# KuldeepChoksi/video-anomaly-detection

Measured on AMD Instinct MI355X. Metric: frames/sec/GPU (256x256 autoencoder scoring) + AUROC parity vs reference, higher is better.
Workload: dtype f32; 1 GPU; configs[1]: image autoencoder scoring, batch 512 synthetic 256x256x3 frames per GPU; chunk=512, weights=deterministic synthetic state dict (Xavier scale, randomised BN), collective=none (1 GPU)

## Files before the change

### video-anomaly-detection_amd/csrc/conv_wino.hip

```cpp
#include <atomic>

#include "vad_common.h"

#define MFMA32W(a, b, c) __builtin_amdgcn_mfma_f32_32x32x2f32((a), (b), (c), 0, 0, 0)

struct ConvWP {
    const float* in;  long long in_fs;
    const float* in2; long long in2_fs;
    int cin_a;
    const float* w;
    const float* bias;
    float* out;       long long out_fs;
    int n, h, w_, cin, cout;
    int tiles_x, tiles_y, cblocks;
    const float* c_prev; float* c_out; int hid;
};

template <int NT, int POOL, int ACT>
__global__ __launch_bounds__(256, 2) void conv3x3_wino_pkernel(ConvWP p) {
    static_assert(POOL != 2 || NT == 2, "fused ConvLSTM cell: two N-tiles (i|f and g|o) per wave");
    constexpr int CK = 32, LW = 18, LH = 10, PS = CK + 4, NPIX = LW * LH;
    constexpr int TOT = NPIX * (CK / 4), NPF = (TOT + 255) / 256;
    constexpr int XF = 4 * 2 * NT * 64 * 16;
    constexpr int TILE_F = NPIX * PS;
    constexpr int SMEM = (2 * TILE_F > XF) ? 2 * TILE_F : XF;
    constexpr int NS = 16;
    constexpr int PB = 1, NB = 2;
    __shared__ __attribute__((aligned(16))) float smem[SMEM];

    const int tid = threadIdx.x, lane = tid & 63, wave = tid >> 6;
    const int li = lane & 31, lh = lane >> 5;

    const unsigned per_frame = (unsigned)(p.tiles_x * p.tiles_y * p.cblocks);
    unsigned L = vad_xcd_remap(blockIdx.x % per_frame, per_frame);
    const int fg = blockIdx.x / per_frame, fgroups = gridDim.x / per_frame;
    const int cb = L % p.cblocks; L /= p.cblocks;
    const int x0 = (L % p.tiles_x) * 16, y0 = (L / p.tiles_x) * 8;
    const int H = p.h, W = p.w_;
    const int nch_a = p.cin_a / CK;
    const int nch = (p.in2 ? p.cin : p.cin_a) / CK;

    unsigned svo[NPF];
    const int c4 = tid & 7, pix0 = tid >> 3;
#pragma unroll
    for (int i = 0; i < NPF; ++i) {
        const int pix = pix0 + 32 * i;
        const int ly = pix / LW, lx = pix - ly * LW;
        const int gy = y0 - 1 + ly, gx = x0 - 1 + lx;
        const bool ok = pix < NPIX && gy >= 0 && gy < H && gx >= 0 && gx < W;
        svo[i] = ok ? (unsigned)(__mul24(__mul24(gy, W) + gx, p.cin_a) + c4 * 4) * 4u : VAD_OOB;
    }
    const unsigned in_bytes = (unsigned)(H * W) * (unsigned)p.cin_a * 4u;
    f32x4 pf[NPF];
#define ISSUE(n_, ch_)                                                                                   \
    {                                                                                                    \
        const float* src_ = ((ch_) < nch_a) ? p.in + (size_t)(n_) * p.in_fs + (ch_) * CK                 \
                                            : p.in2 + (size_t)(n_) * p.in2_fs + ((ch_) - nch_a) * CK;    \
        const unsigned skip_ = (unsigned)(((ch_) < nch_a) ? (ch_) : (ch_) - nch_a) * CK * 4u;            \
        const __amdgpu_buffer_rsrc_t r_ = vad_rsrc(src_, in_bytes - skip_);                              \
        _Pragma("unroll") for (int i_ = 0; i_ < NPF; ++i_) pf[i_] = vad_bload4(r_, svo[i_], 0);          \
    }

    const int tr = li >> 3, tc = li & 7;
    const int ia = (wave == 0) ? 0 : (wave == 2) ? 2 : 1;
    const int ib = (wave == 0) ? 2 : (wave == 1) ? 2 : (wave == 2) ? 1 : 3;
    const float sgn = (wave == 1) ? 1.f : -1.f;
    const int rowa = ((2 * tr + ia) * LW + 2 * tc) * PS + 4 * lh;
    const int rowb = ((2 * tr + ib) * LW + 2 * tc) * PS + 4 * lh;

    const unsigned wf = (unsigned)p.cout * 32u;
    const unsigned ftap = (unsigned)(p.cin / 8) * wf;
    const __amdgpu_buffer_rsrc_t rw = vad_rsrc(p.w, 16u * ftap);
    unsigned wl[NT];
    float bv[NT];
#pragma unroll
    for (int nt = 0; nt < NT; ++nt) {
        const int co = (POOL == 2) ? (2 * nt + (li >> 4)) * p.hid + cb * 16 + (li & 15) : (cb * NT + nt) * 32 + li;
        wl[nt] = (unsigned)(wave * 4) * ftap + (unsigned)co * 32u + 16u * lh;
        bv[nt] = p.bias[co];
    }
    f32x4 b[NB][NT];
#define LOAD_B(buf, chunk, step)                                                 \
    {                                                                                                    \
        const unsigned soff_ = (unsigned)((step) & 3) * ftap + (unsigned)((chunk) * 4 + ((step) >> 2)) * wf; \
        _Pragma("unroll") for (int nt = 0; nt < NT; ++nt) b[buf][nt] = vad_bload4(rw, wl[nt], soff_);    \
    }

    const int ech = (POOL == 2) ? p.hid : p.cout;
    const int ow = (POOL == 1) ? (W >> 1) : W, oh = (POOL == 1) ? (H >> 1) : H;
    const int ey0 = (POOL == 1) ? (y0 >> 1) + wave : y0 + 2 * wave;
    const int ex0 = (POOL == 1) ? (x0 >> 1) + 4 * lh : x0 + 8 * lh;
    const unsigned erow = (unsigned)__mul24(ow, ech) * 4u, ecol = (unsigned)ech * 4u;
    const unsigned eoff = (POOL == 2) ? (unsigned)(__mul24(__mul24(ey0, ow) + ex0 + (li >> 4), ech) + cb * 16 + (li & 15)) * 4u
                                      : (unsigned)(__mul24(__mul24(ey0, ow) + ex0, ech) + cb * NT * 32 + li) * 4u;
    const unsigned out_bytes = (unsigned)__mul24(oh, ow) * (unsigned)ech * 4u;
    const bool full_tile = (y0 + 8 <= H) && (x0 + 16 <= W);
    const int sw = (lane >> 2) & 3;

    int n = fg;
    if (n >= p.n) return;
    ISSUE(n, 0);
#pragma unroll
    for (int s0 = 0; s0 < PB; ++s0) LOAD_B(s0, 0, s0);
#pragma unroll
    for (int nt = 0; nt < NT; ++nt) asm volatile("" ::"v"(bv[nt]));

    f32x16 acc[4][NT];
    const f32x16 zero16 = {0.f, 0.f, 0.f, 0.f, 0.f, 0.f, 0.f, 0.f, 0.f, 0.f, 0.f, 0.f, 0.f, 0.f, 0.f, 0.f};
#define LOAD_RAW(kg)                                                                                     \
    {                                                                                                    \
        _Pragma("unroll") for (int j_ = 0; j_ < 4; ++j_) {                                               \
            raw[0][j_] = *(const f32x4*)&tile_[rowa + j_ * PS + (kg) * 8];                               \
            raw[1][j_] = *(const f32x4*)&tile_[rowb + j_ * PS + (kg) * 8];                               \
        }                                                                                                \
    }
#define TRANSFORM_V()                                                                                    \
    {                                                                                                    \
        f32x4 t_[4];                                                                                     \
        _Pragma("unroll") for (int j_ = 0; j_ < 4; ++j_)                                                 \
            _Pragma("unroll") for (int e_ = 0; e_ < 4; ++e_) t_[j_][e_] = __builtin_fmaf(sgn, raw[1][j_][e_], raw[0][j_][e_]); \
        v[0] = t_[0] - t_[2];                                                                            \
        v[1] = t_[1] + t_[2];                                                                            \
        v[2] = t_[2] - t_[1];                                                                            \
        v[3] = t_[1] - t_[3];                                                                            \
    }
#define CHUNK(FIRST, ch, n_, nn_, has_next_)                                                             \
    {                                                                                                    \
                                       \
        float* tile_ = smem + (((ch) & 1) ? TILE_F : 0);                                                 \
        _Pragma("unroll") for (int i = 0; i < NPF; ++i)                                                  \
            if (pix0 + 32 * i < NPIX) *(f32x4*)&tile_[(pix0 + 32 * i) * PS + c4 * 4] = pf[i];            \
        __syncthreads();                                                                                 \
        f32x4 raw[2][4], v[4];                                 \
        LOAD_RAW(0);                                                                                     \
        if ((ch) + 1 < nch) { ISSUE(n_, (ch) + 1); }                                                     \
        else if (has_next_) { ISSUE(nn_, 0); }                                                           \
        TRANSFORM_V();                                                                                   \
        _Pragma("unroll") for (int kg = 0; kg < 4; ++kg) {                                               \
            if (kg + 1 < 4) { LOAD_RAW(kg + 1); }                                                        \
            _Pragma("unroll") for (int fc = 0; fc < 4; ++fc) {                                           \
                const int s_ = kg * 4 + fc, bcur = s_ % NB, bnxt = (s_ + PB) % NB;                       \
                if (s_ + PB < NS) { LOAD_B(bnxt, ch, s_ + PB); }                                         \
                else if ((ch) + 1 < nch) { LOAD_B(bnxt, (ch) + 1, s_ + PB - NS); }                       \
                __builtin_amdgcn_sched_barrier(0);                                                       \
                _Pragma("unroll") for (int j = 0; j < 4; ++j)                                            \
                    _Pragma("unroll") for (int nt = 0; nt < NT; ++nt)                                    \
                        acc[fc][nt] = MFMA32W(v[fc][j], b[bcur][nt][j], ((FIRST) && kg == 0 && j == 0) ? zero16 : acc[fc][nt]); \
                __builtin_amdgcn_sched_barrier(0);                                                       \
            }                                                                                            \
            if (kg + 1 < 4) { TRANSFORM_V(); }                                                           \
        }                                                                                                \
    }

    while (true) {
        const int nn = n + fgroups;
        const bool has_next = nn < p.n;
        CHUNK(1, 0, n, nn, has_next);
        for (int ch = 1; ch < nch; ++ch) CHUNK(0, ch, n, nn, has_next);

        f32x16 P[2][NT];
#pragma unroll
        for (int nt = 0; nt < NT; ++nt) {
            P[0][nt] = acc[0][nt] + acc[1][nt] + acc[2][nt];
            P[1][nt] = acc[1][nt] - acc[2][nt] - acc[3][nt];
        }
        if (has_next) {
#pragma unroll
            for (int s0 = 0; s0 < PB; ++s0) LOAD_B(s0, 0, s0);
        }
        __syncthreads();
#pragma unroll
        for (int j = 0; j < 2; ++j)
#pragma unroll
            for (int nt = 0; nt < NT; ++nt)
#pragma unroll
                for (int q = 0; q < 4; ++q)
                    *(f32x4*)&smem[((((wave * 2 + j) * NT + nt) * 64 + lane) * 4 + (q ^ sw)) * 4] =
                        f32x4{P[j][nt][4 * q], P[j][nt][4 * q + 1], P[j][nt][4 * q + 2], P[j][nt][4 * q + 3]};
        __syncthreads();
        const __amdgpu_buffer_rsrc_t ro = vad_rsrc(p.out + (size_t)n * p.out_fs, out_bytes);
        f32x4 yy[NT][2][2];
        float cpv[POOL == 2 ? 8 : 1];
        if constexpr (POOL == 2) {
            const __amdgpu_buffer_rsrc_t rc = vad_rsrc(p.c_prev ? p.c_prev + (size_t)n * (out_bytes / 4) : p.c_out, p.c_prev ? out_bytes : 0u);
#pragma unroll
            for (int dy = 0; dy < 2; ++dy)
#pragma unroll
                for (int kk = 0; kk < 4; ++kk) {
                    const bool ok = full_tile || ((ey0 + dy) < oh && (ex0 + 2 * kk + (li >> 4)) < ow);
                    cpv[dy * 4 + kk] = vad_bload1(rc, ok ? eoff : VAD_OOB, dy * erow + 2 * kk * ecol);
                }
        }
#pragma unroll
        for (int nt = 0; nt < NT; ++nt)
#pragma unroll
            for (int j = 0; j < 2; ++j) {
                f32x4 pr[4];
#pragma unroll
                for (int r = 0; r < 4; ++r) pr[r] = *(const f32x4*)&smem[((((r * 2 + j) * NT + nt) * 64 + lane) * 4 + (wave ^ sw)) * 4];
                yy[nt][0][j] = pr[0] + pr[1] + pr[2];
                yy[nt][1][j] = pr[1] - pr[2] - pr[3];
            }
        if constexpr (POOL == 2) {
            const bool hi = (li >> 4) != 0;
            const __amdgpu_buffer_rsrc_t rco = vad_rsrc(p.c_out + (size_t)n * (out_bytes / 4), out_bytes);
#pragma unroll
            for (int dy = 0; dy < 2; ++dy)
#pragma unroll
                for (int kk = 0; kk < 4; ++kk) {
                    float own[2], got[2];
#pragma unroll
                    for (int nt = 0; nt < 2; ++nt) {
                        const float keep = hi ? yy[nt][dy][1][kk] : yy[nt][dy][0][kk];
                        const float give = hi ? yy[nt][dy][0][kk] : yy[nt][dy][1][kk];
                        own[nt] = keep + bv[nt];
                        got[nt] = __builtin_bit_cast(float, __builtin_amdgcn_ds_swizzle(__builtin_bit_cast(int, give + bv[nt]), 0x401f));
                    }
                    const float zi = hi ? got[0] : own[0], zf = hi ? own[0] : got[0], zg = hi ? got[1] : own[1], zo = hi ? own[1] : got[1];
                    float cn, hn;
                    vad_lstm_cell(zi, zf, zg, zo, cpv[dy * 4 + kk], cn, hn);
                    const bool ok = full_tile || ((ey0 + dy) < oh && (ex0 + 2 * kk + (li >> 4)) < ow);
                    const unsigned so = dy * erow + 2 * kk * ecol;
                    vad_bstore1(cn, rco, ok ? eoff : VAD_OOB, so);
                    vad_bstore1(hn, ro, ok ? eoff : VAD_OOB, so);
                }
        } else {
#pragma unroll
            for (int nt = 0; nt < NT; ++nt) {
                if (POOL == 1) {
#pragma unroll
                    for (int kk = 0; kk < 4; ++kk) {
                        const bool ok = full_tile || (ey0 < oh && (ex0 + kk) < ow);
                        const float m = fmaxf(fmaxf(yy[nt][0][0][kk], yy[nt][0][1][kk]), fmaxf(yy[nt][1][0][kk], yy[nt][1][1][kk]));
                        vad_bstore1(vad_act(m + bv[nt], ACT), ro, ok ? eoff : VAD_OOB, kk * ecol + nt * 128u);
                    }
                } else {
#pragma unroll
                    for (int dy = 0; dy < 2; ++dy)
#pragma unroll
                        for (int kk = 0; kk < 4; ++kk)
#pragma unroll
                            for (int dx = 0; dx < 2; ++dx) {
                                const bool ok = full_tile || ((ey0 + dy) < oh && (ex0 + 2 * kk + dx) < ow);
                                vad_bstore1(vad_act(yy[nt][dy][dx][kk] + bv[nt], ACT), ro, ok ? eoff : VAD_OOB, dy * erow + (2 * kk + dx) * ecol + nt * 128u);
                            }
                }
            }
        }
        if (!has_next) break;
        n = nn;
        __syncthreads();
    }
#undef ISSUE
#undef LOAD_B
#undef CHUNK
#undef LOAD_RAW
#undef TRANSFORM_V
}

static int wino_num_cus() {
    static std::atomic<int> cached{0};
    int ncu = cached.load(std::memory_order_relaxed);
    if (!ncu) {
        int dev = 0;
        hipDeviceProp_t prop;
        if (hipGetDevice(&dev) == hipSuccess && hipGetDeviceProperties(&prop, dev) == hipSuccess) ncu = prop.multiProcessorCount;
        if (ncu <= 0) ncu = 256;
        cached = ncu;
    }
    return ncu;
}

template <int NT, int POOL, int ACT>
static void launch_wino(const ConvWP& p, hipStream_t s) {
    static std::atomic<unsigned> cap_{0};
    unsigned cap = cap_.load(std::memory_order_relaxed);
    if (!cap) {
        int per_cu = 0;
        if (hipOccupancyMaxActiveBlocksPerMultiprocessor(&per_cu, conv3x3_wino_pkernel<NT, POOL, ACT>, 256, 0) != hipSuccess || per_cu < 1) per_cu = 1;
        cap_ = cap = (unsigned)wino_num_cus() * (unsigned)per_cu;
    }
    const unsigned per_frame = (unsigned)(p.tiles_x * p.tiles_y * p.cblocks);
    unsigned fgroups = cap / per_frame;
    if (fgroups < 1) fgroups = 1;
    if (fgroups > (unsigned)p.n) fgroups = (unsigned)p.n;
    hipLaunchKernelGGL((conv3x3_wino_pkernel<NT, POOL, ACT>), dim3(per_frame * fgroups), dim3(256), 0, s, p);
}

template <int NT>
static int launch_wino_nt(const ConvWP& p, int act, int pool, hipStream_t s) {
#define W_(P_, A_) launch_wino<NT, P_, A_>(p, s)
    if (pool) { if (act == VAD_ACT_LEAKY) W_(1, VAD_ACT_LEAKY); else if (act == VAD_ACT_RELU) W_(1, VAD_ACT_RELU); else W_(1, VAD_ACT_NONE); }
    else { if (act == VAD_ACT_LEAKY) W_(0, VAD_ACT_LEAKY); else if (act == VAD_ACT_RELU) W_(0, VAD_ACT_RELU); else W_(0, VAD_ACT_NONE); }
#undef W_
    VAD_LAUNCH_CHECK();
    return VAD_OK;
}

#define TRYW(call) do { int rc_ = (call); if (rc_ != VAD_OK) return rc_; } while (0)

extern "C" int vad_conv3x3_wino(const float* in, long long in_fs, const float* w, const float* bias, float* out, long long out_fs,
                                int n, int h, int wd, int cin, int cout, int act, int pool, void* stream) {
    VAD_REQUIRE(in && w && bias && out, "conv3x3_wino: null pointer");
    VAD_REQUIRE(n > 0 && h > 0 && wd > 0, "conv3x3_wino: bad shape n=%d h=%d w=%d", n, h, wd);
    VAD_REQUIRE(cin % 32 == 0 && cout % 32 == 0 && cin > 0 && cout > 0, "conv3x3_wino: cin=%d cout=%d must be positive multiples of 32", cin, cout);
    VAD_REQUIRE(!pool || (h % 2 == 0 && wd % 2 == 0), "conv3x3_wino: pooling needs even H, W (got %dx%d)", h, wd);
    VAD_REQUIRE(act >= 0 && act <= 2, "conv3x3_wino: bad act %d", act);
    const long long chmax = cin > cout ? cin : cout;
    VAD_REQUIRE((long long)h * wd * chmax * 4 < (1ll << 31) && 16ll * cin * cout * 4 < (1ll << 31),
                "conv3x3_wino: frame %dx%dx%lld or weights %dx%d too large for 32-bit offsets", h, wd, chmax, cin, cout);
    ConvWP p{};
    p.in = in; p.in_fs = in_fs ? in_fs : (long long)h * wd * cin; p.cin_a = cin;
    p.w = w; p.bias = bias; p.out = out;
    const int ho = pool ? h / 2 : h, wo = pool ? wd / 2 : wd;
    p.out_fs = out_fs ? out_fs : (long long)ho * wo * cout;
    p.n = n; p.h = h; p.w_ = wd; p.cin = cin; p.cout = cout;
    p.tiles_x = (wd + 15) / 16; p.tiles_y = (h + 7) / 8;
    const bool two = cout % 64 == 0 && (long long)n * p.tiles_x * p.tiles_y * (cout / 64) >= wino_num_cus();
    p.cblocks = cout / (two ? 64 : 32);
    VAD_REQUIRE((long long)p.tiles_x * p.tiles_y * p.cblocks < (1ll << 24), "conv3x3_wino: %d x %d x %d work-group positions out of range", p.tiles_x, p.tiles_y, p.cblocks);
    return two ? launch_wino_nt<2>(p, act, pool, (hipStream_t)stream) : launch_wino_nt<1>(p, act, pool, (hipStream_t)stream);
}

struct CellP {
    const float* z; const float* c_prev; float* c_out; float* h_out;
    long long h_fs;
    int hw, hid;
    long long total;
};

__global__ __launch_bounds__(256) void wino_lstm_cell_kernel(CellP p) {
    const int hq = p.hid >> 2;
    for (long long idx = (long long)blockIdx.x * 256 + threadIdx.x; idx < p.total; idx += (long long)gridDim.x * 256) {
        const long long pix = idx / hq;
        const int c4 = (int)(idx - pix * hq) * 4;
        const long long n = pix / p.hw;
        const int q = (int)(pix - n * p.hw);
        const float* z = p.z + pix * 4 * p.hid + c4;
        const f32x4 zi = *(const f32x4*)z, zf = *(const f32x4*)(z + p.hid), zg = *(const f32x4*)(z + 2 * p.hid), zo = *(const f32x4*)(z + 3 * p.hid);
        const f32x4 cp = p.c_prev ? *(const f32x4*)(p.c_prev + pix * p.hid + c4) : f32x4{0.f, 0.f, 0.f, 0.f};
        f32x4 cn, hn;
#pragma unroll
        for (int e = 0; e < 4; ++e) {
            float c1, h1;
            vad_lstm_cell(zi[e], zf[e], zg[e], zo[e], cp[e], c1, h1);
            cn[e] = c1; hn[e] = h1;
        }
        *(f32x4*)(p.c_out + pix * p.hid + c4) = cn;
        *(f32x4*)(p.h_out + n * p.h_fs + (long long)q * p.hid + c4) = hn;
    }
}

extern "C" int vad_convlstm_step_wino(const float* x, long long x_fs, const float* h_prev, long long h_prev_fs, const float* c_prev,
                                      const float* w, const float* bias, float* h_out, long long h_out_fs, float* c_out, float* z_ws,
                                      int n, int h, int wd, int cin_x, int hid, void* stream) {
    VAD_REQUIRE(x && w && bias && h_out && c_out && z_ws, "convlstm_step_wino: null pointer");
    VAD_REQUIRE((h_prev == nullptr) == (c_prev == nullptr), "convlstm_step_wino: h_prev and c_prev must both be given or both NULL");
    VAD_REQUIRE(n > 0 && h > 0 && wd > 0, "convlstm_step_wino: bad shape %d x %dx%d", n, h, wd);
    VAD_REQUIRE(cin_x > 0 && hid > 0 && hid % 16 == 0 && cin_x % 32 == 0 && cin_x == hid,
                "convlstm_step_wino: cin_x=%d and hid=%d must be equal multiples of 32 (one set of staging offsets serves both sources)", cin_x, hid);
    const int cin = cin_x + hid, cout = 4 * hid;
    VAD_REQUIRE((long long)h * wd * cout * 4 < (1ll << 31) && 16ll * cin * cout * 4 < (1ll << 31), "convlstm_step_wino: frame or weights too large for 32-bit offsets");
    ConvWP p{};
    p.in = x; p.in_fs = x_fs ? x_fs : (long long)h * wd * cin_x; p.cin_a = cin_x;
    p.in2 = h_prev; p.in2_fs = h_prev_fs ? h_prev_fs : (long long)h * wd * hid;
    p.w = w; p.bias = bias; p.out = z_ws; p.out_fs = (long long)h * wd * cout;
    p.n = n; p.h = h; p.w_ = wd; p.cin = cin; p.cout = cout;
    p.tiles_x = (wd + 15) / 16; p.tiles_y = (h + 7) / 8;
    const bool two = (long long)n * p.tiles_x * p.tiles_y * (cout / 64) >= wino_num_cus();
    if (two) {
        p.cblocks = hid / 16; p.hid = hid;
        p.out = h_out; p.out_fs = h_out_fs ? h_out_fs : (long long)h * wd * hid;
        p.c_prev = c_prev; p.c_out = c_out;
        VAD_REQUIRE((long long)p.tiles_x * p.tiles_y * p.cblocks < (1ll << 24), "convlstm_step_wino: grid out of range");
        launch_wino<2, 2, VAD_ACT_NONE>(p, (hipStream_t)stream);
        VAD_LAUNCH_CHECK();
        return VAD_OK;
    }
    p.cblocks = cout / 32;
    TRYW(launch_wino_nt<1>(p, VAD_ACT_NONE, 0, (hipStream_t)stream));
    CellP c{};
    c.z = z_ws; c.c_prev = c_prev; c.c_out = c_out; c.h_out = h_out;
    c.h_fs = h_out_fs ? h_out_fs : (long long)h * wd * hid;
    c.hw = h * wd; c.hid = hid; c.total = (long long)n * h * wd * (hid / 4);
    const long long blocks = (c.total + 255) / 256;
    hipLaunchKernelGGL(wino_lstm_cell_kernel, dim3((unsigned)(blocks < 8192 ? blocks : 8192)), dim3(256), 0, (hipStream_t)stream, c);
    VAD_LAUNCH_CHECK();
    return VAD_OK;
}
```

Measured before the change: 17210 frames/s.

## Cut register pressure in Winograd conv epilogue and weight addressing

Replaces the per-N-tile weight offset arrays with a base offset plus a computed stride, and pins loop-invariant scalars in SGPRs with empty asm constraints. The epilogue now computes the output-transform partial sums one at a time as it writes them to shared memory, and recomputes lane and wave indices from tid. Stores are split into a full-tile fast path and an edge path that uses branchless OOB masking. The goal is lower VGPR pressure and less boundary-check work at two waves per SIMD, at the cost of more complex code and reliance on compiler register allocation.

```diff
diff --git a/video-anomaly-detection_amd/csrc/conv_wino.hip b/video-anomaly-detection_amd/csrc/conv_wino.hip
--- a/video-anomaly-detection_amd/csrc/conv_wino.hip
+++ b/video-anomaly-detection_amd/csrc/conv_wino.hip
@@ -1,4 +1,5 @@
 #include <atomic>
+#include <type_traits>
 
 #include "vad_common.h"
 
@@ -54,9 +55,9 @@
     f32x4 pf[NPF];
 #define ISSUE(n_, ch_)                                                                                   \
     {                                                                                                    \
-        const float* src_ = ((ch_) < nch_a) ? p.in + (size_t)(n_) * p.in_fs + (ch_) * CK                 \
-                                            : p.in2 + (size_t)(n_) * p.in2_fs + ((ch_) - nch_a) * CK;    \
-        const unsigned skip_ = (unsigned)(((ch_) < nch_a) ? (ch_) : (ch_) - nch_a) * CK * 4u;            \
+        const float* src_ = ((ch_) < nch_a_c) ? p.in + (size_t)(n_) * p.in_fs + (ch_) * CK               \
+                                            : p.in2 + (size_t)(n_) * p.in2_fs + ((ch_) - nch_a_c) * CK;  \
+        const unsigned skip_ = (unsigned)(((ch_) < nch_a_c) ? (ch_) : (ch_) - nch_a_c) * CK * 4u;        \
         const __amdgpu_buffer_rsrc_t r_ = vad_rsrc(src_, in_bytes - skip_);                              \
         _Pragma("unroll") for (int i_ = 0; i_ < NPF; ++i_) pf[i_] = vad_bload4(r_, svo[i_], 0);          \
     }
@@ -71,19 +72,20 @@
     const unsigned wf = (unsigned)p.cout * 32u;
     const unsigned ftap = (unsigned)(p.cin / 8) * wf;
     const __amdgpu_buffer_rsrc_t rw = vad_rsrc(p.w, 16u * ftap);
-    unsigned wl[NT];
+    const unsigned co0 = (POOL == 2) ? (li >> 4) * p.hid + cb * 16 + (li & 15) : cb * NT * 32 + li;
+    const unsigned cont = (POOL == 2) ? 2u * (unsigned)p.hid : 32u;
+    const unsigned wl = (unsigned)(wave * 4) * ftap + co0 * 32u + 16u * lh;
+    const unsigned wl1 = wl + cont * 32u;
     float bv[NT];
 #pragma unroll
-    for (int nt = 0; nt < NT; ++nt) {
-        const int co = (POOL == 2) ? (2 * nt + (li >> 4)) * p.hid + cb * 16 + (li & 15) : (cb * NT + nt) * 32 + li;
-        wl[nt] = (unsigned)(wave * 4) * ftap + (unsigned)co * 32u + 16u * lh;
-        bv[nt] = p.bias[co];
-    }
+    for (int nt = 0; nt < NT; ++nt) bv[nt] = p.bias[co0 + nt * cont];
     f32x4 b[NB][NT];
+    unsigned ftap_c = ftap, wf_c = wf;
+    int nch_c = nch, nch_a_c = nch_a;
 #define LOAD_B(buf, chunk, step)                                                 \
     {                                                                                                    \
-        const unsigned soff_ = (unsigned)((step) & 3) * ftap + (unsigned)((chunk) * 4 + ((step) >> 2)) * wf; \
-        _Pragma("unroll") for (int nt = 0; nt < NT; ++nt) b[buf][nt] = vad_bload4(rw, wl[nt], soff_);    \
+        const unsigned soff_ = (unsigned)((step) & 3) * ftap_c + (unsigned)((chunk) * 4 + ((step) >> 2)) * wf_c; \
+        _Pragma("unroll") for (int nt = 0; nt < NT; ++nt) b[buf][nt] = vad_bload4(rw, (POOL == 2) ? (nt ? wl1 : wl) : wl + nt * 1024u, soff_); \
     }
 
     const int ech = (POOL == 2) ? p.hid : p.cout;
@@ -94,8 +96,6 @@
     const unsigned eoff = (POOL == 2) ? (unsigned)(__mul24(__mul24(ey0, ow) + ex0 + (li >> 4), ech) + cb * 16 + (li & 15)) * 4u
                                       : (unsigned)(__mul24(__mul24(ey0, ow) + ex0, ech) + cb * NT * 32 + li) * 4u;
     const unsigned out_bytes = (unsigned)__mul24(oh, ow) * (unsigned)ech * 4u;
-    const bool full_tile = (y0 + 8 <= H) && (x0 + 16 <= W);
-    const int sw = (lane >> 2) & 3;
 
     int n = fg;
     if (n >= p.n) return;
@@ -128,12 +128,14 @@
     {                                                                                                    \
                                        \
         float* tile_ = smem + (((ch) & 1) ? TILE_F : 0);                                                 \
+                                    \
+        asm volatile("" : "+s"(ftap_c), "+s"(wf_c), "+s"(nch_c), "+s"(nch_a_c));                         \
         _Pragma("unroll") for (int i = 0; i < NPF; ++i)                                                  \
             if (pix0 + 32 * i < NPIX) *(f32x4*)&tile_[(pix0 + 32 * i) * PS + c4 * 4] = pf[i];            \
         __syncthreads();                                                                                 \
         f32x4 raw[2][4], v[4];                                 \
         LOAD_RAW(0);                                                                                     \
-        if ((ch) + 1 < nch) { ISSUE(n_, (ch) + 1); }                                                     \
+        if ((ch) + 1 < nch_c) { ISSUE(n_, (ch) + 1); }                                                   \
         else if (has_next_) { ISSUE(nn_, 0); }                                                           \
         TRANSFORM_V();                                                                                   \
         _Pragma("unroll") for (int kg = 0; kg < 4; ++kg) {                                               \
@@ -141,7 +143,7 @@
             _Pragma("unroll") for (int fc = 0; fc < 4; ++fc) {                                           \
                 const int s_ = kg * 4 + fc, bcur = s_ % NB, bnxt = (s_ + PB) % NB;                       \
                 if (s_ + PB < NS) { LOAD_B(bnxt, ch, s_ + PB); }                                         \
-                else if ((ch) + 1 < nch) { LOAD_B(bnxt, (ch) + 1, s_ + PB - NS); }                       \
+                else if ((ch) + 1 < nch_c) { LOAD_B(bnxt, (ch) + 1, s_ + PB - NS); }                     \
                 __builtin_amdgcn_sched_barrier(0);                                                       \
                 _Pragma("unroll") for (int j = 0; j < 4; ++j)                                            \
                     _Pragma("unroll") for (int nt = 0; nt < NT; ++nt)                                    \
@@ -158,95 +160,110 @@
         CHUNK(1, 0, n, nn, has_next);
         for (int ch = 1; ch < nch; ++ch) CHUNK(0, ch, n, nn, has_next);
 
-        f32x16 P[2][NT];
-#pragma unroll
-        for (int nt = 0; nt < NT; ++nt) {
-            P[0][nt] = acc[0][nt] + acc[1][nt] + acc[2][nt];
-            P[1][nt] = acc[1][nt] - acc[2][nt] - acc[3][nt];
-        }
         if (has_next) {
 #pragma unroll
             for (int s0 = 0; s0 < PB; ++s0) LOAD_B(s0, 0, s0);
         }
         __syncthreads();
-#pragma unroll
-        for (int j = 0; j < 2; ++j)
-#pragma unroll
-            for (int nt = 0; nt < NT; ++nt)
+        unsigned et = (unsigned)tid;
+        if constexpr (NT == 2) asm volatile("" : "+v"(et));
+        const unsigned el = et & 63u, ew = et >> 6, sw = (el >> 2) & 3u;
+        const unsigned wrec = ((ew * (2 * NT * 64) + el) * 4 + sw) * 4;
+        const unsigned rrec = (el * 4 + (ew ^ sw)) * 4;
+#pragma unroll
+        for (int nt = 0; nt < NT; ++nt)
+#pragma unroll
+            for (int j = 0; j < 2; ++j) {
+                const f32x16 P = j ? acc[1][nt] - acc[2][nt] - acc[3][nt] : acc[0][nt] + acc[1][nt] + acc[2][nt];
 #pragma unroll
                 for (int q = 0; q < 4; ++q)
-                    *(f32x4*)&smem[((((wave * 2 + j) * NT + nt) * 64 + lane) * 4 + (q ^ sw)) * 4] =
-                        f32x4{P[j][nt][4 * q], P[j][nt][4 * q + 1], P[j][nt][4 * q + 2], P[j][nt][4 * q + 3]};
+                    *(f32x4*)&smem[(wrec ^ (4 * q)) + (j * NT + nt) * 1024] = f32x4{P[4 * q], P[4 * q + 1], P[4 * q + 2], P[4 * q + 3]};
+            }
         __syncthreads();
+        unsigned erow_t = erow, ecol_t = ecol, eoff_t = eoff;
+        asm volatile("" : "+s"(erow_t), "+s"(ecol_t));
+        if constexpr (NT == 2) asm volatile("" : "+v"(eoff_t));
         const __amdgpu_buffer_rsrc_t ro = vad_rsrc(p.out + (size_t)n * p.out_fs, out_bytes);
-        f32x4 yy[NT][2][2];
-        float cpv[POOL == 2 ? 8 : 1];
-        if constexpr (POOL == 2) {
-            const __amdgpu_buffer_rsrc_t rc = vad_rsrc(p.c_prev ? p.c_prev + (size_t)n * (out_bytes / 4) : p.c_out, p.c_prev ? out_bytes : 0u);
-#pragma unroll
-            for (int dy = 0; dy < 2; ++dy)
-#pragma unroll
-                for (int kk = 0; kk < 4; ++kk) {
-                    const bool ok = full_tile || ((ey0 + dy) < oh && (ex0 + 2 * kk + (li >> 4)) < ow);
-                    cpv[dy * 4 + kk] = vad_bload1(rc, ok ? eoff : VAD_OOB, dy * erow + 2 * kk * ecol);
+        auto finish = [&](auto fullc) {
+            constexpr bool FULL = decltype(fullc)::value;
+            unsigned er = et;
+            if constexpr (!FULL) asm volatile("" : "+v"(er));
+            const int elh = (er >> 5) & 1, eli = er & 31;
+            const int ey_ = (POOL == 1) ? (y0 >> 1) + (int)(er >> 6) : y0 + 2 * (int)(er >> 6);
+            const int ex_ = (POOL == 1) ? (x0 >> 1) + 4 * elh : (POOL == 2) ? x0 + 8 * elh + (eli >> 4) : x0 + 8 * elh;
+            auto vo = [&](int dy, int dx) {
+                if constexpr (FULL) return eoff_t;
+                else return eoff_t | ((unsigned)((oh - 1 - dy - ey_) | (ow - 1 - dx - ex_)) & VAD_OOB);
+            };
+            auto row_half = [&](int nt, f32x4 (&y)[2][2]) {
+#pragma unroll
+                for (int j = 0; j < 2; ++j) {
+                    f32x4 pr[4];
+#pragma unroll
+                    for (int r = 0; r < 4; ++r) pr[r] = *(const f32x4*)&smem[rrec + ((r * 2 + j) * NT + nt) * 1024];
+                    y[0][j] = pr[0] + pr[1] + pr[2];
+                    y[1][j] = pr[1] - pr[2] - pr[3];
                 }
-        }
-#pragma unroll
-        for (int nt = 0; nt < NT; ++nt)
-#pragma unroll
-            for (int j = 0; j < 2; ++j) {
-                f32x4 pr[4];
-#pragma unroll
-                for (int r = 0; r < 4; ++r) pr[r] = *(const f32x4*)&smem[((((r * 2 + j) * NT + nt) * 64 + lane) * 4 + (wave ^ sw)) * 4];
-                yy[nt][0][j] = pr[0] + pr[1] + pr[2];
-                yy[nt][1][j] = pr[1] - pr[2] - pr[3];
-            }
-        if constexpr (POOL == 2) {
-            const bool hi = (li >> 4) != 0;
-            const __amdgpu_buffer_rsrc_t rco = vad_rsrc(p.c_out + (size_t)n * (out_bytes / 4), out_bytes);
-#pragma unroll
-            for (int dy = 0; dy < 2; ++dy)
-#pragma unroll
-                for (int kk = 0; kk < 4; ++kk) {
-                    float own[2], got[2];
-#pragma unroll
-                    for (int nt = 0; nt < 2; ++nt) {
-                        const float keep = hi ? yy[nt][dy][1][kk] : yy[nt][dy][0][kk];
-                        const float give = hi ? yy[nt][dy][0][kk] : yy[nt][dy][1][kk];
-                        own[nt] = keep + bv[nt];
-                        got[nt] = __builtin_bit_cast(float, __builtin_amdgcn_ds_swizzle(__builtin_bit_cast(int, give + bv[nt]), 0x401f));
+            };
+            if constexpr (POOL == 2) {
+                const __amdgpu_buffer_rsrc_t rc = vad_rsrc(p.c_prev ? p.c_prev + (size_t)n * (out_bytes / 4) : p.c_out, p.c_prev ? out_bytes : 0u);
+                float cpv[8];
+#pragma unroll
+                for (int dy = 0; dy < 2; ++dy)
+#pragma unroll
+                    for (int kk = 0; kk < 4; ++kk)
+                        cpv[dy * 4 + kk] = vad_bload1(rc, vo(dy, 2 * kk), dy * erow_t + 2 * kk * ecol_t);
+                f32x4 yy[2][2][2];
+                row_half(0, yy[0]);
+                row_half(1, yy[1]);
+                const bool hi = (li >> 4) != 0;
+                const __amdgpu_buffer_rsrc_t rco = vad_rsrc(p.c_out + (size_t)n * (out_bytes / 4), out_bytes);
+#pragma unroll
+                for (int dy = 0; dy < 2; ++dy)
+#pragma unroll
+                    for (int kk = 0; kk < 4; ++kk) {
+                        float own[2], got[2];
+#pragma unroll
+                        for (int nt = 0; nt < 2; ++nt) {
+                            const float keep = hi ? yy[nt][dy][1][kk] : yy[nt][dy][0][kk];
+                            const float give = hi ? yy[nt][dy][0][kk] : yy[nt][dy][1][kk];
+                            own[nt] = keep + bv[nt];
+                            got[nt] = __builtin_bit_cast(float, __builtin_amdgcn_ds_swizzle(__builtin_bit_cast(int, give + bv[nt]), 0x401f));
+                        }
+                        const float zi = hi ? got[0] : own[0], zf = hi ? own[0] : got[0], zg = hi ? got[1] : own[1], zo = hi ? own[1] : got[1];
+                        float cn, hn;
+                        vad_lstm_cell(zi, zf, zg, zo, cpv[dy * 4 + kk], cn, hn);
+                        const unsigned v = vo(dy, 2 * kk), so = dy * erow_t + 2 * kk * ecol_t;
+                        vad_bstore1(cn, rco, v, so);
+                        vad_bstore1(hn, ro, v, so);
                     }
-                    const float zi = hi ? got[0] : own[0], zf = hi ? own[0] : got[0], zg = hi ? got[1] : own[1], zo = hi ? own[1] : got[1];
-                    float cn, hn;
-                    vad_lstm_cell(zi, zf, zg, zo, cpv[dy * 4 + kk], cn, hn);
-                    const bool ok = full_tile || ((ey0 + dy) < oh && (ex0 + 2 * kk + (li >> 4)) < ow);
-                    const unsigned so = dy * erow + 2 * kk * ecol;
-                    vad_bstore1(cn, rco, ok ? eoff : VAD_OOB, so);
-                    vad_bstore1(hn, ro, ok ? eoff : VAD_OOB, so);
-                }
-        } else {
-#pragma unroll
-            for (int nt = 0; nt < NT; ++nt) {
-                if (POOL == 1) {
-#pragma unroll
-                    for (int kk = 0; kk < 4; ++kk) {
-                        const bool ok = full_tile || (ey0 < oh && (ex0 + kk) < ow);
-                        const float m = fmaxf(fmaxf(yy[nt][0][0][kk], yy[nt][0][1][kk]), fmaxf(yy[nt][1][0][kk], yy[nt][1][1][kk]));
-                        vad_bstore1(vad_act(m + bv[nt], ACT), ro, ok ? eoff : VAD_OOB, kk * ecol + nt * 128u);
+            } else {
+#pragma unroll
+                for (int nt = 0; nt < NT; ++nt) {
+                    f32x4 y[2][2];
+                    row_half(nt, y);
+                    if (POOL == 1) {
+#pragma unroll
+                        for (int kk = 0; kk < 4; ++kk) {
+                            const float m = fmaxf(fmaxf(y[0][0][kk], y[0][1][kk]), fmaxf(y[1][0][kk], y[1][1][kk]));
+                            vad_bstore1(vad_act(m + bv[nt], ACT), ro, vo(0, kk) + nt * 128u, kk * ecol_t);
+                        }
+                    } else {
+#pragma unroll
+                        for (int dy = 0; dy < 2; ++dy)
+#pragma unroll
+                            for (int kk = 0; kk < 4; ++kk)
+#pragma unroll
+                                for (int dx = 0; dx < 2; ++dx)
+                                    vad_bstore1(vad_act(y[dy][dx][kk] + bv[nt], ACT), ro, vo(dy, 2 * kk + dx) + nt * 128u,
+                                                dy * erow_t + (2 * kk + dx) * ecol_t);
                     }
-                } else {
-#pragma unroll
-                    for (int dy = 0; dy < 2; ++dy)
-#pragma unroll
-                        for (int kk = 0; kk < 4; ++kk)
-#pragma unroll
-                            for (int dx = 0; dx < 2; ++dx) {
-                                const bool ok = full_tile || ((ey0 + dy) < oh && (ex0 + 2 * kk + dx) < ow);
-                                vad_bstore1(vad_act(yy[nt][dy][dx][kk] + bv[nt], ACT), ro, ok ? eoff : VAD_OOB, dy * erow + (2 * kk + dx) * ecol + nt * 128u);
-                            }
                 }
             }
-        }
+        };
+        int y0_t = y0;
+        asm volatile("" : "+s"(y0_t));
+        if (y0_t + 8 <= H && x0 + 16 <= W) finish(std::true_type{}); else finish(std::false_type{});
         if (!has_next) break;
         n = nn;
         __syncthreads();
```

New measurement: 17240 frames/s (median of 4 runs). About the same (+0.2%).
